# adaliaramon/LambdaGap

Measured on AMD Instinct MI355X. Metric: boosting iters/sec + AUC, synthetic Higgs-shape 10M×28, 255 bins, 63 leaves, higher is better.
Workload: dtype fp32; 1 GPU; model=gbdt binary, 63 leaves, 255 bins, lr 0.1, global_batch=10000000, seq_len=28, parallelism=dp1, device=AMD GPU (gfx950:sramecc+:xnack-) [frontier engine]

## Files before the change

src/device/device_learner.hip:

```cpp
#include <hip/hip_runtime.h>

#include <algorithm>
#include <chrono>
#include <cmath>
#include <cstdio>
#include <cstdlib>
#include <cstring>
#include <fstream>
#include <map>
#include <memory>
#include <string>
#include <vector>

#include "device/grad_kernels.h"
#include "device/hip_common.h"
#include "device/leaf_kernels.h"
#include "device/metric_kernels.h"
#include "device/linear_kernels.h"
#include "device/runtime_internal.h"
#include "device/frontier.h"
#include "device/policy_scan.h"
#include "device/traverse_kernels.h"
#include "device/sample_kernels.h"
#include "device/engine_plan.h"
#include "device/seq_kernels.h"
#include "device/split_scan.h"
#include "device/tree_kernels.h"
#include "learner/forced_splits.h"
#include "learner/linear_solve.h"
#include "learner/parallel_tree_learner.h"
#include "learner/serial_tree_learner.h"
#include "lgap/common.h"
#include "lgap/device_api.h"
#include "lgap/network.h"
#include "lgap/objective.h"
#include "lgap/rank_math.h"
#include "lgap/metric.h"
#include "lgap/split_math.h"

namespace lgap {
namespace device {
namespace {

const char* KernelOverride(const char* key) {
  static const char* const kKeys[] = {"fhist_threads", "hist_lds_kb", "quant_lds32", "part_iters",
                                      "hist_il",       "nibble",      "quant_hist",  "scan_global",
                                      "scan_wave",     "oob_rows",    "select_merge"};
  constexpr int kNumKeys = static_cast<int>(sizeof(kKeys) / sizeof(kKeys[0]));
  thread_local std::string vals[kNumKeys];
  const char* e = std::getenv("LGAP_KERNEL");
  if (e == nullptr) return nullptr;
  const std::string s(e);
  const char* found = nullptr;
  for (size_t p = 0; p < s.size();) {
    size_t q = s.find(',', p);
    if (q == std::string::npos) q = s.size();
    const std::string item = s.substr(p, q - p);
    p = q + 1;
    if (item.empty()) continue;
    const size_t eq = item.find('=');
    const std::string k = item.substr(0, eq);
    int idx = -1;
    for (int i = 0; i < kNumKeys; ++i) idx = k == kKeys[i] ? i : idx;
    if (idx < 0) Log::Fatal("LGAP_KERNEL: unknown key '%s'", k.c_str());
    if (k == key) {
      vals[idx] = eq == std::string::npos ? "1" : item.substr(eq + 1);
      found = vals[idx].c_str();
    }
  }
  return found;
}


using namespace seq;

template <typename T>
class PinnedBuf {
 public:
  ~PinnedBuf() {
    if (p_) (void)hipHostFree(p_);
// ... 1597 lines not shown
      facc_recv_.Resize(static_cast<size_t>(K) * bbin_ * 2);
    }
    if (plan_.bynode_on_device) {
      bool filt = false;
      const std::vector<uint8_t> m = col_sampler_.ByNodeSampleModes(&fbyn_cnt_, &filt);
      fbyn_reset_ = filt ? 1 : 0;
      fbyn_mode_.Resize(m.size());
      fbyn_mode_.Upload(m.data(), m.size(), stream_);
    }
    if (fvoting_) {
      SplitParams sl = MakeArgs().sp;
      sl.min_data_in_leaf = config_->min_data_in_leaf / P_;
      sl.min_sum_hessian_in_leaf = config_->min_sum_hessian_in_leaf / P_;
      fsp_local_.Resize(1);
      fsp_local_.Upload(&sl, 1, stream_);
      flsum_loc_.Resize(C);
      fltot_.Resize(2 * K);
      fltot_.Zero(stream_);
      fvrec_.Resize(static_cast<size_t>(P_) * 2 * K * topk_);
      fvelect_.Resize(2 * K * static_cast<size_t>(topk_ + 1));
      fvrows_.Resize(2 * K * static_cast<size_t>(topk_) * 2 * max_bin_);
    }
    fpart_iters_ = part_iters_;
    fpart_tile_ = kPartThreads * fpart_iters_;
    ftile_cap_ = DivUp(N_, fpart_tile_) + fkmax_ + 1;
    ftile_pub_.Resize(ftile_cap_);
    ftile_pub_.Zero(stream_);
    for (int i = 3; i < kFrontierIdx; ++i) idx_[i].Resize(std::max(N_, 1));
    {
      const int per_cu = std::max(1, FrontierPartitionBlocksPerCU(fpart_iters_));
      fpart_grid_ = std::max(1, std::min(ftile_cap_, per_cu * num_cu_));
    }
    fscan_lds_ = FrontierScanLds(max_bin_, has_cat_ ? max_cat_bin_ : 1);
    FrontierSetLds(FrontierHistLds(), fscan_lds_, use_dp_, width_);
    fspec_cap_ = 0;
    fhist_threads_ = big_tiles_ || (num_tiles_ == 1 && N_ >= 4000000) ? 1024 : 512;
    if (const char* e = KernelOverride("fhist_threads")) fhist_threads_ = std::atoi(e) == 1024 ? 1024 : 512;
    fpolicy_ = 1;
    fspec_alpha_ = 1.0;
    const char* spec_env = std::getenv("LGAP_FRONTIER_SPEC");
    const std::string spec = spec_env != nullptr ? spec_env : "";
    fspec_fixed_ = spec != "adapt";
    if (!spec.empty() && spec != "adapt" && spec != "fixed") {
      char* end = nullptr;
      const double alpha = std::strtod(spec.c_str(), &end);
      if (end == spec.c_str() || *end != '\0') Log::Fatal("LGAP_FRONTIER_SPEC=%s: expected fixed|adapt|<alpha>", spec.c_str());
      fspec_alpha_ = std::max(0.01, std::min(4.0, alpha));
    }
    {
      stune_ = SpecTuner();
      const char* te = std::getenv("LGAP_SPEC_TUNE");
      const bool tune_small = te == nullptr || te[0] != '0';
      stune_.on = !plan_.distributed && (L_ >= 128 || tune_small) && !plan_.raw_cands && fnum_forced_ == 0 &&
                  spec.empty();
      if (L_ < 128 && te == nullptr) stune_.rest = 64;
    }
    if (std::getenv("LGAP_FSTAMPS")) {
      fstamps_.Resize(256 * 4 * kFStampSlots);
      fstamps_.Zero(stream_);
    }
    for (auto& kv : fgraphs_) (void)hipGraphExecDestroy(kv.second);
    fgraphs_.clear();
    if (fcont_) (void)hipGraphExecDestroy(fcont_);
    fcont_ = nullptr;
  }

  FArgs MakeFArgs() const {
    FArgs a;
    std::memset(&a, 0, sizeof(a));
    a.rowbins = rowbins_.get();
// ... 58 lines not shown
    if (nib_) {
      a.rowbins = rowbins4_.get();
      a.stride_dw = stride4_dw_;
      a.tiles = ntile_.get();
      a.hist_nib = 1;
    }
    a.part_tile = fpart_tile_;
    a.max_depth = config_->max_depth;
    a.use_monotone = config_->monotone_constraints.empty() ? 0 : 1;
    a.mono_inter = fcbnd_ != nullptr ? 1 : 0;
    a.cbnd = fcbnd_;
    const char* sm = KernelOverride("select_merge");
    a.salive = sm != nullptr && sm[0] == '0' ? nullptr : fsal_;
    a.monotone_penalty = config_->monotone_penalty;
    a.cegb_split = CegbPenalty::Enabled(config_) ? config_->cegb_tradeoff * config_->cegb_penalty_split : 0.0;
    a.max_bin = max_bin_;
    a.cat_p2 = cat_p2_;
    a.use_dp = use_dp_ ? 1 : 0;
    a.ghq = ghq_.get();
    a.qmax = qmax_.get();
    a.quant = QuantHist() && ghq_.size() >= static_cast<size_t>(K_) * N_ ? 1 : 0;
    a.qbins = std::max(2, config_->num_grad_quant_bins);
    a.qconst = is_const_hess_ ? 1 : 0;
    {
      const double rows = static_cast<double>(N_);
      const double gl = a.qbins / 2, hl = a.qconst ? 1 : a.qbins;
      a.qpack = rows * gl < 2147483647.0 && rows * hl < 4294967295.0 ? 1 : 0;
      const int sub = static_cast<int>(std::min(32767.0 / gl, 65535.0 / hl));
      const char* e = KernelOverride("quant_lds32");
      const bool want = e != nullptr ? e[0] != '0' : num_tiles_ == 1;
      a.qsub = a.quant && !use_dp_ && sub >= 2048 && want ? sub : 0;
    }
    a.hist_il = !use_dp_ && a.qsub == 0 ? HistInterleave() : 0;
    {
      const bool fits = kFScanWaves * FrontierScanWaveBytes(max_bin_, cat_p2_) <= 150 * 1024;
      const char* sw = KernelOverride("scan_wave");
      a.scan_wave = fits && !has_cat_ && !a.mono_inter && (F_ >= 64 || (sw != nullptr && sw[0] == '1')) ? 1 : 0;
      a.scan_grid = 512;
    }
    a.e_lo = 0;
    a.e_hi = kFrontierKmax;
    if (plan_.raw_cands && fnuep_.size() > 0) {
      a.cegb_raw = 1;
      a.cegb_tradeoff = config_->cegb_tradeoff;
      a.nkey = fnkey_.get();
      a.ninfo = fninfo_.get();
      a.nuep = fnuep_.get();
      if (plan_.cegb_coupled) {
        a.cegb_coupled = cegb_coupled_.get();
        a.cegb_used = cegb_used_.get();
        a.cegb_epoch = cegb_epoch_.get();
      }
      if (plan_.cegb_lazy) {
        a.cegb_lazy = cegb_lazy_.get();
        a.lazy_bits = lazy_bits_.get();
        a.lazy_words = lazy_words_;
        a.lazy_acc = lazy_acc_.get();
        a.nlazy = fnlazy_.get();
        a.npath = fnpath_.get();
      }
    }
    a.spec_cap = fspec_cap_;
    a.policy = fpolicy_;
    a.stamps = fstamps_.size() ? fstamps_.get() : nullptr;
    a.distributed = plan_.distributed ? 1 : 0;
    a.kcap = fcaps_on_ ? fkcap_.get() : nullptr;
// ... 481 lines not shown
    if (renew && gh_true_.size() < static_cast<size_t>(N_)) gh_true_.Resize(N_);
    qmax_.Zero(stream_);
    const int grid = std::max(1, std::min(DivUp(N_, 256), num_cu_ * 4));
    k_qmax<<<grid, 256, 0, stream_>>>(gh, N_, qmax_.get());
    HIP_CHECK(hipGetLastError());
    if (Network::num_machines() > 1) {
      unsigned* hm = pin_max_.Get(2);
      qmax_.Download(hm, 2, stream_);
      HIP_CHECK(hipStreamSynchronize(stream_));
      float v[2];
      std::memcpy(v, hm, 8);
      v[0] = static_cast<float>(Network::GlobalSyncUpByMax(static_cast<double>(v[0])));
      v[1] = static_cast<float>(Network::GlobalSyncUpByMax(static_cast<double>(v[1])));
      std::memcpy(hm, v, 8);
      HIP_CHECK(hipMemcpyAsync(qmax_.get(), hm, 8, hipMemcpyHostToDevice, stream_));
    }
    const uint32_t seed = static_cast<uint32_t>(config_->seed) * 0x9E3779B9u + (quant_round_++);
    uint16_t* ghq = nullptr;
    if (QuantHist()) {
      if (ghq_.size() < static_cast<size_t>(K_) * N_) {
        ghq_.Resize(static_cast<size_t>(K_) * N_);
        InvalidateGraph();
      }
      ghq = ghq_.get() + static_cast<size_t>(class_id) * N_;
    }
    k_quantize<<<grid, 256, 0, stream_>>>(gh, renew ? gh_true_.get() : nullptr, ghq, N_, qmax_.get(),
                                          std::max(2, config_->num_grad_quant_bins), is_const_hess_ ? 1 : 0, seed,
                                          config_->stochastic_rounding ? 1 : 0);
    HIP_CHECK(hipGetLastError());
  }

  size_t FrontierHistLds() const {
    const FArgs fa = MakeFArgs();
    const size_t plan = use_dp_ || fa.qsub > 0 ? hist_lds_plain_ : hist_lds_bytes_;
    const size_t b = use_dp_ || !QuantHist() || fa.qsub == 0 ? plan : plan * 3 / 2 + 64;
    return b;
  }

  bool QuantHist() const {
    return config_->use_quantized_grad && std::max(2, config_->num_grad_quant_bins) <= 254 &&
           KernelOverride("quant_hist") == nullptr;
  }

  void RenewQuantizedLeaves(Tree* tree) {
    const int nl = tree->num_leaves();
    const Args args = MakeArgs();
    k_leaf_true_sums<<<nl, kNodeThreads, 0, stream_>>>(args, gh_true_.get(), nl, true_sums_.get());
    HIP_CHECK(hipGetLastError());
    std::vector<double2> st(nl);
    true_sums_.Download(st.data(), nl, stream_);
    HIP_CHECK(hipStreamSynchronize(stream_));
    std::vector<double> flat(2 * nl);
    for (int l = 0; l < nl; ++l) flat[2 * l] = st[l].x, flat[2 * l + 1] = st[l].y;
    if (plan_.distributed) Network::GlobalSum(&flat);
    SplitParams p = MakeArgs().sp;
    p.path_smooth = 0.0;
    for (int l = 0; l < nl; ++l) {
      tree->SetLeafOutput(l, LeafOutputRaw(flat[2 * l], flat[2 * l + 1], p, tree->leaf_count(l), 0.0));
    }
  }

  void BackendSetGradients(const float* g, const float* h, int n) {
    if (n != N_) Log::Fatal("HistogramBackend: %d gradients for %d rows", n, N_);
    K_ = 1;
    if (gh_.size() < static_cast<size_t>(N_)) gh_.Resize(static_cast<size_t>(N_));
    DeviceSetGradients(g, h, 1);
    float mg = 0.f, mh = 0.f;
    for (int i = 0; i < N_; ++i) {
      mg = std::max(mg, std::fabs(g[i]));
      mh = std::max(mh, std::fabs(h[i]));
// ... 559 lines not shown
    if (scan_global_) {
      scan_scratch_.Resize(scan_scratch_stride_ * static_cast<size_t>(std::max(F_, 1)));
      Log::Debug("HIP split scan: %d-bin features use %zu bytes of global scratch per block", max_bin_,
                 scan_scratch_stride_);
    } else if (scan_lds_bytes_ > 64 * 1024) {
      HIP_CHECK(hipFuncSetAttribute(reinterpret_cast<const void*>(k_reduce_scan<float, false>),
                                    hipFuncAttributeMaxDynamicSharedMemorySize, static_cast<int>(scan_lds_bytes_)));
      HIP_CHECK(hipFuncSetAttribute(reinterpret_cast<const void*>(k_reduce_scan<double, false>),
                                    hipFuncAttributeMaxDynamicSharedMemorySize, static_cast<int>(scan_lds_bytes_)));
    }
    std::vector<int> gs(std::max(G_, 1));
    for (int g = 0; g < G_; ++g) gs[g] = data_->group(g).hist_start;
    h_gstart_ = gs;
    BuildTiles();
    BuildNibbleRows();
    HIP_CHECK(hipStreamSynchronize(stream_));
  }

  void BuildTiles() {
    row_align_ = RowAlign();
    const int env_kb = [] {
      const char* e = KernelOverride("hist_lds_kb");
      return e ? std::max(16, std::min(150, std::atoi(e))) : 0;
    }();
    big_tiles_ = false;
    PlanTiles(env_kb > 0 ? env_kb * 1024 : kHistLdsBytes);
    if (env_kb == 0 && plan_.mode == ParallelMode::kSerial && num_tiles_ > 1 && min_tile_dw_ < 16) {
      big_tiles_ = true;
      PlanTiles(150 * 1024);
    }
    if (num_tiles_ > 1 && row_align_ > 0) PadTrainingRows(row_align_);
    if (num_tiles_ == 1) {
      if (N_ >= (4 << 20) && stride_dw_ > 4 && stride_dw_ < 8) PadTrainingRows(8);
    }
  }

  void BuildNibbleRows() {
    nib_ = false;
    const char* e = KernelOverride("nibble");
    if (e != nullptr && e[0] == '0') return;
    if (width_ != 1 || num_tiles_ != 1 || G_ <= 0 || N_ <= 0 || h_tiles_.empty() || h_tiles_[0].direct) return;
    for (int g = 0; g < G_; ++g) {
      if (data_->group(g).num_bin > 16) return;
    }
    stride4_dw_ = DivUp(G_, 8);
    rowbins4_.Resize(static_cast<size_t>(N_) * stride4_dw_);
    LaunchPackNibbles(rowbins_.get(), tstride_dw_, N_, G_, rowbins4_.get(), stride4_dw_, stream_);
    HistTile t = h_tiles_[0];
    t.d0 = 0;
    t.d1 = stride4_dw_;
    ntile_.Resize(1);
    ntile_.Upload(&t, 1, stream_);
    HIP_CHECK(hipStreamSynchronize(stream_));
    nib_ = true;
    Log::Debug("HIP learner: 4-bit rows (%d dwords per row instead of %d)", stride4_dw_, stride_dw_);
  }

  void PlanTiles(int lds_budget) {
    const int per = 4 / width_;
    const size_t acc = use_dp_ ? 16 : 8;
    const int max_bins = static_cast<int>(lds_budget / acc) - 64;
    const int max_dw = kHistThreads / 2;
    std::vector<HistTile> tiles;
    hist_lds_bytes_ = 16;
    hist_lds_plain_ = 16;
    int d = 0;
// ... 987 lines not shown
```

src/device/frontier.h:

```cpp
#pragma once

#include <hip/hip_runtime.h>

#include <cstdint>

#include "device/frontier_shape.h"
#include "device/tree_kernels.h"
#include "lgap/split_math.h"

namespace lgap {
namespace device {

#ifndef LGAP_FRONTIER_BUFS
#define LGAP_FRONTIER_BUFS 4
#endif
constexpr int kFrontierBufs = LGAP_FRONTIER_BUFS;
constexpr int kFrontierIdx = kFrontierBufs + 1;
constexpr int kFrontierRoundCap = 64;

__host__ __device__ inline int FixedPointExp(double limit, double rows, float vmax, float vsum) {
  double b = rows * static_cast<double>(vmax);
  if (static_cast<double>(vsum) < b) b = static_cast<double>(vsum);
  if (!(b > 0.0)) return 0;
  int e;
  (void)frexp(limit / b, &e);
  return e - 1;
}

__host__ __device__ inline int FrontierDepthBuf(int j) { return j < 2 ? j : j + 1; }

constexpr uint8_t kNodeExpanded = 1;
constexpr uint8_t kNodeCommitted = 2;
constexpr uint8_t kNodeDead = 4;
constexpr uint8_t kNodeStale = 0x40;
constexpr uint8_t kNodeEligTmp = 0x20;
constexpr uint8_t kNodeRescanTmp = 0x10;
constexpr uint8_t kNodeLocal = 0xF0;
constexpr int kFStampPart = 0, kFStampHist = 1, kFStampScan = 2, kFStampSel = 3, kFStampSlots = 8;

struct FNode {
  int buf, start, count;
  int gcount;
  int depth, parent;
  int left;
  int fidx;
};

struct FPairBest {
  SplitKey key;
  SplitInfo info;
};

struct FForced {
  int feature, threshold, left, right;
};

struct FExp {
  int parent, left, depth;
  int tile0, ntiles;
  int src_buf, start, count;
  int dst_buf;
  int group, offset, num_bin, mfb, default_bin, missing, thr, default_left, is_cat;
  int skip;
  int smaller, larger;
  int h_buf, h_start, h_count;
  int forced;
  int feature;
  int last;
  int rescan;
};

// ... 47 lines not shown
  double* slots;
  unsigned long long* acc;
  unsigned long long* hslab;
  size_t hslab_stride;
  long long* hmeta;
  int red_grid;
  int own, own_P, own_rank, own_w;
  const int* own_b0;
  unsigned long long* acc_recv;
  int xkb;
  const int* fown_list;
  int fown_n;
  const unsigned* ghmax;
  int sum_mult;
  int sum_bound;
  const FForced* forced;
  int num_forced;
  SplitInfo* fbest;
  SplitKey* fkey;
  const uint16_t* ghq;
  const unsigned* qmax;
  int quant;
  int qpack;
  int qbins, qconst;
  int qsub;
  SplitKey* ckey;
  SplitInfo* cinfo;
  unsigned long long* tile_pub;
  unsigned* bar;
  int part_selfcount;
  int hist_min_rows, hist_grid;
  int hist_threads;
  int hist_il;
  int scan_wave;
  int scan_grid;
  int hist_nib;
  int part_tile;
  int max_depth, use_monotone;
  int mono_inter;
  LeafBounds* cbnd;
  int* salive;
  double monotone_penalty;
  double cegb_split;
  const double* cegb_coupled;
  double cegb_tradeoff;
  uint8_t* cegb_used;
  unsigned* cegb_epoch;
  SplitKey* nkey;
  SplitInfo* ninfo;
  int* nuep;
  int cegb_raw;
  const double* cegb_lazy;
  uint32_t* lazy_bits;
  int lazy_words;
  int* lazy_acc;
  int* nlazy;
  uint32_t* npath;
  int max_bin, cat_p2;
  int use_dp;
  int spec_cap;
  int policy;
  int distributed;
  const int* kcap;
  int* kused;
  unsigned long long* stamps;
  int e_lo, e_hi;
// ... 81 lines not shown
```

src/device/frontier_kernels.hip:

```cpp
#include <hip/hip_runtime.h>

#include <algorithm>
#include <cstdint>

#include "device/frontier.h"
#include "device/hip_common.h"
#include "device/split_scan.h"
#include "lgap/split_math.h"

namespace lgap {
namespace device {
namespace {

constexpr int kFPartThreads = 256;
constexpr int kFScanThreads = 256;
constexpr int kFSelThreads = 1024;
#ifndef LGAP_FHIST_R
#define LGAP_FHIST_R 16
#endif

__device__ __forceinline__ int FRowAt(const FArgs& a, int buf, int pos) { return buf < 0 ? pos : a.idx[buf][pos]; }

__device__ __forceinline__ uint32_t FColBin(const FArgs& a, int g, int row) {
  const size_t o = static_cast<size_t>(g) * a.N + row;
  return a.width == 1 ? a.colbins[o] : reinterpret_cast<const uint16_t*>(a.colbins)[o];
}

__device__ __forceinline__ void FStamp(const FArgs& a, int r, int kern, int i) {
  if (a.stamps != nullptr && blockIdx.x == 0 && blockIdx.y == 0 && threadIdx.x == 0) {
    a.stamps[((static_cast<size_t>(r & 255) * 4 + kern) * kFStampSlots) + i] = wall_clock64();
  }
}
__device__ __forceinline__ void FStampMax(const FArgs& a, int r, int kern, int i) {
  if (a.stamps != nullptr && threadIdx.x == 0) {
    atomicMax(&a.stamps[((static_cast<size_t>(r & 255) * 4 + kern) * kFStampSlots) + i], wall_clock64());
  }
}
__device__ __forceinline__ void FStampEnd(const FArgs& a, int r, int kern) {
  if (a.stamps != nullptr && threadIdx.x == 0) {
    atomicMax(&a.stamps[((static_cast<size_t>(r & 255) * 4 + kern) * kFStampSlots) + 7], wall_clock64());
  }
}

__device__ __forceinline__ int Pow2Exp(double x) {
  int e;
  (void)frexp(x, &e);
  return e - 1;
}

__device__ __forceinline__ void GlobalScaleExp(const FArgs& a, int* eg, int* eh) {
  const double n = static_cast<double>(a.tp->root_gcount > 0 ? a.tp->root_gcount : 1);
  constexpr double k62 = 4611686018427387904.0;
  const float m = a.sum_bound ? static_cast<float>(a.sum_mult > 1 ? a.sum_mult : 1) : INFINITY;
  *eg = FixedPointExp(k62, n, __uint_as_float(a.ghmax[0]), __uint_as_float(a.ghmax[2]) * m);
  *eh = FixedPointExp(k62, n, __uint_as_float(a.ghmax[1]), __uint_as_float(a.ghmax[3]) * m);
}

__device__ __forceinline__ void QuantScales(const FArgs& a, double* gs, double* hs) {
// ... 201 lines not shown
#pragma unroll
    for (int j = 0; j < kRootStatsF; ++j) sh[j][w] = v[j];
  }
  __syncthreads();
  if (threadIdx.x == 0) {
    for (int i = 1; i < static_cast<int>(blockDim.x / 64); ++i) {
#pragma unroll
      for (int j = 0; j < kRootStatsF; ++j) v[j] = FRootFold(j, v[j], sh[j][i]);
    }
    a.lsum[0] = make_double2(v[0], v[1]);
    ghmax[0] = __float_as_uint(static_cast<float>(v[2]));
    ghmax[1] = __float_as_uint(static_cast<float>(v[3]));
    ghmax[2] = __float_as_uint(__double2float_ru(v[4] * (1.0 + 0x1p-20)));
    ghmax[3] = __float_as_uint(__double2float_ru(v[5] * (1.0 + 0x1p-20)));
  }
}

constexpr int kFHistR2 = LGAP_FHIST_R / 2;
__device__ __forceinline__ void FHistFirstRows(const FArgs& a, const HistTile& tile, int buf, int start, int rb, int re,
                                               int* rn) {
  const int tpr = tile.d1 - tile.d0;
  const int rpi = blockDim.x / tpr;
  const int myr = threadIdx.x / tpr;
  const int* idx = buf < 0 ? nullptr : a.idx[buf] + start;
  const int base = buf < 0 ? start : 0;
#pragma unroll
  for (int j = 0; j < kFHistR2; ++j) {
    const int p = rb + myr + j * rpi;
    rn[j] = myr < rpi && p < re ? (idx ? idx[p] : base + p) : -1;
  }
}

template <int W, int MODE>
__device__ __forceinline__ void FHistRows(const FArgs& a, const HistTile& tile, int buf, int start, int rb, int re,
                                          const int* gst, unsigned long long* hist, float sg, float sh, double dsg,
                                          double dsh, uint32_t* hist32 = nullptr, int il_gp = 0,
                                          const int* first_rows = nullptr) {
  const int tpr = tile.d1 - tile.d0;
  const int rpi = blockDim.x / tpr;
  const int myr = threadIdx.x / tpr;
  const int myd = threadIdx.x - myr * tpr;
  if (myr >= rpi) return;
  constexpr int per = W == 0 ? 8 : 4 / W;
  constexpr int R = LGAP_FHIST_R;
  const int dw = tile.d0 + myd;
  const int gfirst = dw * per;
  int go[per], gsh[per];
  const int rot = (MODE == 0 || MODE == 2) && il_gp > 0 ? (myr & (per - 1)) : 0;
#pragma unroll
  for (int kk = 0; kk < per; ++kk) {
    int gv = -1, sv = 0;
#pragma unroll
    for (int k = 0; k < per; ++k) {
      if (k == ((kk + rot) & (per - 1))) {
        const int gl = gfirst + k - tile.g0;
        gv = gfirst + k < tile.g1 ? (il_gp > 0 ? gl : gst[gl]) : -1;
        sv = (W == 0 ? 4 : W == 1 ? 8 : 16) * k;
      }
    }
    go[kk] = gv;
    gsh[kk] = sv;
  }
  const float2* gh = a.gh + static_cast<size_t>(a.tp->cls) * a.N;
  const uint16_t* ghq = MODE >= 2 ? a.ghq + static_cast<size_t>(a.tp->cls) * a.N : nullptr;
  const int* idx = buf < 0 ? nullptr : a.idx[buf] + start;
  const int base = buf < 0 ? start : 0;
  constexpr int R2 = R / 2;
  static_assert(R2 == kFHistR2, "first-chunk prefetch width");
  const int step = rpi * R2;
  auto load_rows = [&](int p0, int* rows) {
#pragma unroll
    for (int j = 0; j < R2; ++j) {
      const int p = p0 + j * rpi;
      rows[j] = p < re ? (idx ? idx[p] : base + p) : -1;
    }
  };
  auto load_data = [&](const int* rows, uint32_t* word, float2* v, uint32_t* q) {
#pragma unroll
    for (int j = 0; j < R2; ++j) {
      word[j] = rows[j] >= 0 ? a.rowbins[static_cast<size_t>(rows[j]) * a.stride_dw + dw] : 0u;
      if (MODE >= 2) q[j] = rows[j] >= 0 ? ghq[rows[j]] : 0u;
      else v[j] = rows[j] >= 0 ? gh[rows[j]] : make_float2(0.f, 0.f);
    }
  };
  int rn[R2];
  uint32_t word[R2], q[R2];
  float2 v[R2];
  if (first_rows != nullptr) {
#pragma unroll
    for (int j = 0; j < R2; ++j) rn[j] = first_rows[j];
  } else {
    load_rows(rb + myr, rn);
  }
  load_data(rn, word, v, q);
  load_rows(rb + myr + step, rn);
  for (int p0 = rb + myr; p0 < re; p0 += step) {
    uint32_t wn[R2], qn[R2];
    float2 vn[R2];
    load_data(rn, wn, vn, qn);
    load_rows(p0 + 2 * step, rn);
#pragma unroll
    for (int j = 0; j < R2; ++j) {
      unsigned long long pg = 0ull, ph = 0ull;
      uint32_t p32 = 0u;
      if (MODE == 3) {
        p32 = (static_cast<uint32_t>(static_cast<int32_t>(static_cast<int8_t>(q[j] >> 8))) << 16) + (q[j] & 0xFFu);
      } else if (MODE == 2) {
        const long long ig = static_cast<int8_t>(q[j] >> 8);
        pg = (static_cast<unsigned long long>(ig) << 32) + (q[j] & 0xFFu);
      } else if (MODE == 0) {
        const long long ig = __float2int_rn(v[j].x * sg);
        const long long ih = __float2int_rn(v[j].y * sh);
        pg = (static_cast<unsigned long long>(ig) << 32) + static_cast<unsigned long long>(ih);
      } else {
        pg = static_cast<unsigned long long>(__double2ll_rn(static_cast<double>(v[j].x) * dsg));
        ph = static_cast<unsigned long long>(__double2ll_rn(static_cast<double>(v[j].y) * dsh));
      }
#pragma unroll
      for (int k = 0; k < per; ++k) {
        const uint32_t b = (word[j] >> gsh[k]) & (W == 0 ? 0xFu : W == 1 ? 0xFFu : 0xFFFFu);
        if (b != 0u && go[k] >= 0) {
          const int o = il_gp > 0 ? static_cast<int>(b) * il_gp + go[k] : go[k] + static_cast<int>(b);
          if (MODE == 3) {
            atomicAdd(&hist32[o], p32);
          } else if (MODE != 1) {
            atomicAdd(&hist[o], pg);
          } else {
            atomicAdd(&hist[2 * o], pg);
            atomicAdd(&hist[2 * o + 1], ph);
          }
        }
      }
    }
#pragma unroll
    for (int j = 0; j < R2; ++j) {
      word[j] = wn[j];
      q[j] = qn[j];
      v[j] = vn[j];
    }
  }
}

struct FChunkSrc {
  int cnt, buf, start;
};
__device__ __forceinline__ FChunkSrc FHistChunkLoad(const FArgs& a) {
  FChunkSrc c{0, -1, 0};
  const int t = threadIdx.x;
  if (t < kFrontierKmax) {
    const FExp& x = a.exps[t];
    c.cnt = x.skip ? 0 : x.h_count;
    c.buf = x.h_buf;
    c.start = x.h_start;
  }
  return c;
}
__device__ __forceinline__ void FHistChunks(const FArgs& a, int k, const FChunkSrc& src, int* cnt, int* nb, int* inc) {
  const int t = threadIdx.x;
  *cnt = t < k && t >= a.e_lo && t < a.e_hi ? src.cnt : 0;
  const int total = WaveSum(*cnt);
  const int ke = WaveSum(*cnt > 0 ? 1 : 0);
  const int slots = max(max(1, a.hist_grid / 2), a.hist_grid - ke);
  const int c = max(a.hist_min_rows, (total + slots - 1) / slots);
  *nb = (*cnt + c - 1) / c;
  *inc = WaveInclusiveScan(*nb);
}

template <int W, int MODE, int THREADS>
__global__ __launch_bounds__(THREADS) void k_f_hist(FArgs a) {
  extern __shared__ __align__(8) unsigned char lds_raw[];
  __shared__ int s_e, s_rb, s_re, s_buf, s_start;
  const FState* sp = a.st;
  const int t = threadIdx.x;
  const FChunkSrc csrc = FHistChunkLoad(a);
  const HistTile tile = a.tiles[blockIdx.y];
  const int ng0 = tile.g1 - tile.g0;
  const int gst0 = t < ng0 ? a.gstart[tile.g0 + t] : 0;
  int EG, EH;
  GlobalScaleExp(a, &EG, &EH);
  if (sp->done) return;
  const int k = sp->k;
  const int rnd = sp->round;
  FStamp(a, rnd, kFStampHist, 0);
  if (t < 64) {
    int cnt, nb, inc;
    FHistChunks(a, k, csrc, &cnt, &nb, &inc);
    const int bx = static_cast<int>(blockIdx.x);
    const bool mine = nb > 0 && bx >= inc - nb && bx < inc;
    const unsigned long long m = __ballot(mine);
    if (mine) {
      const int j = bx - (inc - nb);
      const int chunk = (cnt + nb - 1) / nb;
      s_e = t;
      s_rb = j * chunk;
      s_re = min(cnt, (j + 1) * chunk);
      s_buf = csrc.buf;
      s_start = csrc.start;
    }
    if (t == 0 && m == 0ull) s_e = -1;
  }
  __syncthreads();
  const int e = s_e;
  if (e < 0) return;
// ... 55 lines not shown
                           : W == 1 ? ((word >> (8 * kk)) & 0xFFu)
                                    : ((word >> (16 * kk)) & 0xFFFFu);
        const int g = dw * per + kk;
        if (b != 0u && g < tile.g1) {
          unsigned long long* o = FAccPtr(a, e, gst[g - tile.g0] + static_cast<int>(b), pw);
          if (a.xg && a.own) {
            if (qg) FXAdd(o, qg);
            if (qh) FXAdd(o + 1, qh);
          } else {
            if (qg) atomicAdd(o, qg);
            if (qh) atomicAdd(o + 1, qh);
          }
        }
      }
    }
    if (a.xg && a.own) __builtin_amdgcn_s_waitcnt(0);
    return;
  }
  const double rows_in_block = static_cast<double>(re - rb > 0 ? re - rb : 1);
  constexpr double k30 = 1073741824.0;
  const float sbg = a.sum_bound ? __uint_as_float(a.ghmax[2]) : INFINITY;
  const float sbh = a.sum_bound ? __uint_as_float(a.ghmax[3]) : INFINITY;
  const int bg = FixedPointExp(k30, rows_in_block, __uint_as_float(a.ghmax[0]), sbg);
  const int bh = FixedPointExp(k30, rows_in_block, __uint_as_float(a.ghmax[1]), sbh);
  const float sg = ldexpf(1.f, bg), sh = ldexpf(1.f, bh);
  const int ng = tile.g1 - tile.g0;
  const int il_gp = (MODE == 0 || MODE == 2) && a.hist_il && tile.pad > 0 && (buf < 0 || a.hist_il > 1) ? ((ng + 15) & ~15) : 0;
  const int words = il_gp > 0 ? tile.pad * il_gp : (MODE != 1 ? tile.nbins : 2 * tile.nbins);
  unsigned long long* hist = reinterpret_cast<unsigned long long*>(lds_raw);
  uint32_t* hist32 = reinterpret_cast<uint32_t*>(hist + words);
  int* gst = reinterpret_cast<int*>(MODE == 3 ? reinterpret_cast<unsigned long long*>(hist32 + ((tile.nbins + 1) & ~1))
                                              : hist + words);
  unsigned long long* packed = il_gp > 0 ? reinterpret_cast<unsigned long long*>(gst + ((ng + 1) & ~1)) : nullptr;
  int first_rows[kFHistR2];
  if (MODE != 3) FHistFirstRows(a, tile, buf, start, rb, re, first_rows);
  for (int i = t; i < words; i += blockDim.x) hist[i] = 0ull;
  if (MODE == 3) {
    for (int i = t; i < tile.nbins; i += blockDim.x) hist32[i] = 0u;
  }
  for (int g = t; g < ng0; g += blockDim.x) gst[g] = (g == t ? gst0 : a.gstart[tile.g0 + g]) - tile.bin0;
  __syncthreads();
  FStamp(a, rnd, kFStampHist, 1);
  if (MODE == 3) {
    for (int sb = rb; sb < re; sb += a.qsub) {
      const int se = min(re, sb + a.qsub);
      FHistRows<W, MODE>(a, tile, buf, start, sb, se, gst, hist, sg, sh, dsg, dsh, hist32);
      __syncthreads();
      for (int i = t; i < tile.nbins; i += blockDim.x) {
        const uint32_t x = hist32[i];
        if (x == 0u) continue;
        hist32[i] = 0u;
        const uint32_t hs = x & 0xFFFFu;
        const long long gs = static_cast<int32_t>(x - hs) >> 16;
        hist[i] += (static_cast<unsigned long long>(gs) << 32) + hs;
      }
      __syncthreads();
    }
  } else {
    FHistRows<W, MODE>(a, tile, buf, start, rb, re, gst, hist, sg, sh, dsg, dsh, nullptr, il_gp, first_rows);
    __syncthreads();
  }
  if (il_gp > 0) {
    for (int sl = t; sl < words; sl += blockDim.x) {
      const int b = sl / il_gp, gl = sl - b * il_gp;
      if (gl >= ng) continue;
      const int nb = (gl + 1 < ng ? gst[gl + 1] : tile.nbins) - gst[gl];
      if (b < nb) packed[gst[gl] + b] = hist[sl];
    }
    __syncthreads();
  }
  FStamp(a, rnd, kFStampHist, 2);
  FStampMax(a, rnd, kFStampHist, 5);
  const int sw = MODE == 1 ? 2 : 1;
  unsigned long long* prow = a.hslab + static_cast<size_t>(blockIdx.x) * a.hslab_stride + static_cast<size_t>(sw) * tile.bin0;
  const unsigned long long* src = il_gp > 0 ? packed : hist;
  for (int j = t; j < sw * tile.nbins; j += blockDim.x) prow[j] = src[j];
  if (MODE == 0 && t == 0) {
    a.hmeta[blockIdx.x] = static_cast<long long>((static_cast<unsigned long long>(static_cast<unsigned>(bh)) << 32) |
                                                 static_cast<unsigned>(bg));
  }
  FStamp(a, rnd, kFStampHist, 3);
  FStampMax(a, rnd, kFStampHist, 6);
  FStampEnd(a, rnd, kFStampHist);
}

constexpr int kRedThreads = 256;
constexpr int kRedRows = 16;
constexpr int kRedMaxTiles = 256;

template <int MODE, bool XG>
__global__ __launch_bounds__(kRedThreads) void k_f_reduce(FArgs a) {
  __shared__ int s_nb[kFrontierKmax], s_b0[kFrontierKmax], s_w0[kFrontierKmax + 1];
// ... 433 lines not shown
        kk.feature = out->feature;
        kk.gain = SafeGain(*out);
        kk.threshold = out->threshold;
        kk.group = fi.group;
        kk.offset = fi.offset;
        kk.num_bin = fi.num_bin;
        kk.mfb = fi.mfb;
        kk.default_bin = fi.default_bin;
        kk.missing = fi.missing;
        kk.default_left = out->default_left;
        kk.is_cat = fi.bin_type != 0 ? 1 : 0;
        kk.pad0 = a.cegb_raw && out->feature >= 0 ? out->monotone_type : 0;
      }
    }
    __syncthreads();
    if (item == static_cast<int>(blockIdx.x)) FStamp(a, rnd, kFStampScan, 2);
    constexpr int kKeyWords = static_cast<int>(sizeof(SplitKey) / 4);
    constexpr int kInfoWords = static_cast<int>(sizeof(SplitInfo) / 4);
    const int nsel = cl >= 0 ? 2 : 1;
    for (int i = t; i < nsel * (kKeyWords + kInfoWords); i += blockDim.x) {
      const int sel = i / (kKeyWords + kInfoWords);
      const int o = i - sel * (kKeyWords + kInfoWords);
      const size_t q = (static_cast<size_t>(e) * 2 + sel) * F + f;
      if (o < kKeyWords) {
        reinterpret_cast<uint32_t*>(a.ckey + q)[o] = reinterpret_cast<const uint32_t*>(&s_key[sel])[o];
      } else {
        reinterpret_cast<uint32_t*>(a.cinfo + q)[o - kKeyWords] = reinterpret_cast<const uint32_t*>(&s_out[sel])[o - kKeyWords];
      }
    }
    __syncthreads();
    if (item == static_cast<int>(blockIdx.x)) FStamp(a, rnd, kFStampScan, 3);
  }
  FStampEnd(a, rnd, kFStampScan);
}

__device__ __forceinline__ void FWaveSync() {
  __builtin_amdgcn_fence(__ATOMIC_RELEASE, "workgroup");
  __builtin_amdgcn_wave_barrier();
  __builtin_amdgcn_fence(__ATOMIC_ACQUIRE, "workgroup");
}

__global__ __launch_bounds__(kFScanWaves * 64) void k_f_scan_w(FArgs a) {
  extern __shared__ __align__(16) unsigned char smem[];
  __shared__ __align__(8) unsigned char s_out_raw[kFScanWaves * sizeof(SplitInfo)];
  __shared__ SplitKey s_key[kFScanWaves];
  const FState* stp = a.st;
  if (stp->done) return;
  const int e0 = a.e_lo, e1 = min(stp->k, a.e_hi), F = a.F;
  const int total = max(0, e1 - e0) * F;
  const int rnd = stp->round;
  FStamp(a, rnd, kFStampScan, 0);
  const int t = threadIdx.x, lane = t & 63, w = t >> 6;
  int EG, EH;
  GlobalScaleExp(a, &EG, &EH);
  double inv_g = ldexp(1.0, -EG), inv_h = ldexp(1.0, -EH);
  if (a.quant) QuantScales(a, &inv_g, &inv_h);
  const bool qpack = a.quant && a.qpack;
  const size_t TB2 = 2 * static_cast<size_t>(a.TB);
  double* hs_full = reinterpret_cast<double*>(smem + w * FrontierScanWaveBytes(a.max_bin, a.cat_p2));
  double* hl_full = hs_full + 2 * a.max_bin;
  SplitInfo* out = reinterpret_cast<SplitInfo*>(s_out_raw) + w;
  SplitKey* key = &s_key[w];
  constexpr int kKeyWords = static_cast<int>(sizeof(SplitKey) / 4);
  constexpr int kInfoWords = static_cast<int>(sizeof(SplitInfo) / 4);
  for (int item = static_cast<int>(blockIdx.x) * kFScanWaves + w; item < total;
       item += static_cast<int>(gridDim.x) * kFScanWaves) {
    const int e = e0 + item / F, f = item - (e - e0) * F;
    const FExp& xr = a.exps[e];
    if (xr.skip) continue;
    const int cs = xr.smaller, cl = xr.larger, p = xr.parent;
    const DevFeature fi = a.feat[f];
    const int nbin = fi.num_bin;
// ... 2699 lines not shown
```

Baseline: 390.3 iters/s.

## Stage histogram row loads through per-wave LDS ring with 16-byte vector loads

Adds a staged histogram path for 8-bit bins in which each wave's lanes cooperatively load whole row segments as 16-byte vectors, plus gradient/hessian pairs, into a per-wave LDS ring. The lanes then read their own bin word from LDS and do the atomic adds, with wave-level fences between the two phases. Loads are software-pipelined with depth D. The aim is to replace narrow, poorly coalesced per-thread global loads of row bins with wide coalesced ones, at the cost of extra LDS space, wave syncs and possibly lower occupancy. It is on by default for single-tile datasets with at least 4M rows, which matches this workload.

After: 393.8 iters/s, median of 6. Within noise of the previous version (+0.9%).

```diff
diff --git a/src/device/device_learner.hip b/src/device/device_learner.hip
--- a/src/device/device_learner.hip
+++ b/src/device/device_learner.hip
@@ -45,7 +45,7 @@
 const char* KernelOverride(const char* key) {
   static const char* const kKeys[] = {"fhist_threads", "hist_lds_kb", "quant_lds32", "part_iters",
                                       "hist_il",       "nibble",      "quant_hist",  "scan_global",
-                                      "scan_wave",     "oob_rows",    "select_merge"};
+                                      "scan_wave",     "oob_rows",    "select_merge", "hist_stage"};
   constexpr int kNumKeys = static_cast<int>(sizeof(kKeys) / sizeof(kKeys[0]));
   thread_local std::string vals[kNumKeys];
   const char* e = std::getenv("LGAP_KERNEL");
@@ -1709,10 +1709,10 @@
       fpart_grid_ = std::max(1, std::min(ftile_cap_, per_cu * num_cu_));
     }
     fscan_lds_ = FrontierScanLds(max_bin_, has_cat_ ? max_cat_bin_ : 1);
-    FrontierSetLds(FrontierHistLds(), fscan_lds_, use_dp_, width_);
     fspec_cap_ = 0;
     fhist_threads_ = big_tiles_ || (num_tiles_ == 1 && N_ >= 4000000) ? 1024 : 512;
     if (const char* e = KernelOverride("fhist_threads")) fhist_threads_ = std::atoi(e) == 1024 ? 1024 : 512;
+    FrontierSetLds(FrontierHistLds(), fscan_lds_, use_dp_, width_);
     fpolicy_ = 1;
     fspec_alpha_ = 1.0;
     const char* spec_env = std::getenv("LGAP_FRONTIER_SPEC");
@@ -1837,6 +1837,7 @@
       a.qsub = a.quant && !use_dp_ && sub >= 2048 && want ? sub : 0;
     }
     a.hist_il = !use_dp_ && a.qsub == 0 ? HistInterleave() : 0;
+    a.hist_stage = HistStage(a.qsub) ? 1 : 0;
     {
       const bool fits = kFScanWaves * FrontierScanWaveBytes(max_bin_, cat_p2_) <= 150 * 1024;
       const char* sw = KernelOverride("scan_wave");
@@ -2384,10 +2385,26 @@
 
   size_t FrontierHistLds() const {
     const FArgs fa = MakeFArgs();
-    const size_t plan = use_dp_ || fa.qsub > 0 ? hist_lds_plain_ : hist_lds_bytes_;
-    const size_t b = use_dp_ || !QuantHist() || fa.qsub == 0 ? plan : plan * 3 / 2 + 64;
+    return FrontierHistLdsPlan(fa.qsub) + (fa.hist_stage ? FrontierHistStageLds(fhist_threads_) : 0);
+  }
+  size_t FrontierHistLdsPlan(int qsub) const {
+    const size_t plan = use_dp_ || qsub > 0 ? hist_lds_plain_ : hist_lds_bytes_;
+    const size_t b = use_dp_ || !QuantHist() || qsub == 0 ? plan : plan * 3 / 2 + 64;
     return b;
   }
+
+  bool HistStage(int qsub) const {
+    const char* e = KernelOverride("hist_stage");
+    if (e != nullptr && e[0] == '0') return false;
+    if (nib_ || width_ != 1 || tstride_dw_ % 4 != 0) return false;
+    constexpr size_t kCuLds = 160 * 1024, kBlockLds = 159 * 1024;
+    const size_t plan = FrontierHistLdsPlan(qsub), with = plan + FrontierHistStageLds(fhist_threads_);
+    if (with > kBlockLds) return false;
+    if (num_tiles_ > 1 && std::min<size_t>(kCuLds / with, 2) < std::min<size_t>(kCuLds / plan, 2)) return false;
+    if (e != nullptr) return true;
+    return HistStageDefault();
+  }
+  bool HistStageDefault() const { return num_tiles_ == 1 && N_ >= (4 << 20) && !use_dp_; }
 
   bool QuantHist() const {
     return config_->use_quantized_grad && std::max(2, config_->num_grad_quant_bins) <= 254 &&
@@ -3013,6 +3030,9 @@
     if (num_tiles_ > 1 && row_align_ > 0) PadTrainingRows(row_align_);
     if (num_tiles_ == 1) {
       if (N_ >= (4 << 20) && stride_dw_ > 4 && stride_dw_ < 8) PadTrainingRows(8);
+    }
+    if (const char* e = KernelOverride("hist_stage")) {
+      if (e[0] != '0' && width_ == 1 && tstride_dw_ % 4 != 0) PadTrainingRows(4);
     }
   }
 
diff --git a/src/device/frontier.h b/src/device/frontier.h
--- a/src/device/frontier.h
+++ b/src/device/frontier.h
@@ -37,6 +37,12 @@
 constexpr uint8_t kNodeRescanTmp = 0x10;
 constexpr uint8_t kNodeLocal = 0xF0;
 constexpr int kFStampPart = 0, kFStampHist = 1, kFStampScan = 2, kFStampSel = 3, kFStampSlots = 8;
+#ifndef LGAP_FHIST_STAGE_D
+#define LGAP_FHIST_STAGE_D 2
+#endif
+constexpr int kFHistStageD = LGAP_FHIST_STAGE_D;
+constexpr int kFHistStageWaveBytes = 1024 + 512;
+constexpr size_t FrontierHistStageLds(int threads) { return 32 + static_cast<size_t>(threads / 64) * kFHistStageWaveBytes; }
 
 struct FNode {
   int buf, start, count;
@@ -150,6 +156,7 @@
   int hist_min_rows, hist_grid;
   int hist_threads;
   int hist_il;
+  int hist_stage;
   int scan_wave;
   int scan_grid;
   int hist_nib;
diff --git a/src/device/frontier_kernels.hip b/src/device/frontier_kernels.hip
--- a/src/device/frontier_kernels.hip
+++ b/src/device/frontier_kernels.hip
@@ -24,6 +24,12 @@
 __device__ __forceinline__ uint32_t FColBin(const FArgs& a, int g, int row) {
   const size_t o = static_cast<size_t>(g) * a.N + row;
   return a.width == 1 ? a.colbins[o] : reinterpret_cast<const uint16_t*>(a.colbins)[o];
+}
+
+__device__ __forceinline__ void FWaveSync() {
+  __builtin_amdgcn_fence(__ATOMIC_RELEASE, "workgroup");
+  __builtin_amdgcn_wave_barrier();
+  __builtin_amdgcn_fence(__ATOMIC_ACQUIRE, "workgroup");
 }
 
 __device__ __forceinline__ void FStamp(const FArgs& a, int r, int kern, int i) {
@@ -291,6 +297,65 @@
 }
 
 template <int W, int MODE>
+__device__ __forceinline__ void FHistGroups(const HistTile& tile, const int* gst, int il_gp, int myr, int dw, int* go,
+                                            int* gsh) {
+  constexpr int per = W == 0 ? 8 : 4 / W;
+  const int gfirst = dw * per;
+  const int rot = (MODE == 0 || MODE == 2) && il_gp > 0 ? (myr & (per - 1)) : 0;
+#pragma unroll
+  for (int kk = 0; kk < per; ++kk) {
+    int gv = -1, sv = 0;
+#pragma unroll
+    for (int k = 0; k < per; ++k) {
+      if (k == ((kk + rot) & (per - 1))) {
+        const int gl = gfirst + k - tile.g0;
+        gv = gfirst + k < tile.g1 ? (il_gp > 0 ? gl : gst[gl]) : -1;
+        sv = (W == 0 ? 4 : W == 1 ? 8 : 16) * k;
+      }
+    }
+    go[kk] = gv;
+    gsh[kk] = sv;
+  }
+}
+
+template <int W, int MODE>
+__device__ __forceinline__ void FHistAdd(uint32_t word, float2 v, uint32_t q, const int* go, const int* gsh,
+                                         unsigned long long* hist, uint32_t* hist32, int il_gp, float sg, float sh,
+                                         double dsg, double dsh) {
+  constexpr int per = W == 0 ? 8 : 4 / W;
+  unsigned long long pg = 0ull, ph = 0ull;
+  uint32_t p32 = 0u;
+  if (MODE == 3) {
+    p32 = (static_cast<uint32_t>(static_cast<int32_t>(static_cast<int8_t>(q >> 8))) << 16) + (q & 0xFFu);
+  } else if (MODE == 2) {
+    const long long ig = static_cast<int8_t>(q >> 8);
+    pg = (static_cast<unsigned long long>(ig) << 32) + (q & 0xFFu);
+  } else if (MODE == 0) {
+    const long long ig = __float2int_rn(v.x * sg);
+    const long long ih = __float2int_rn(v.y * sh);
+    pg = (static_cast<unsigned long long>(ig) << 32) + static_cast<unsigned long long>(ih);
+  } else {
+    pg = static_cast<unsigned long long>(__double2ll_rn(static_cast<double>(v.x) * dsg));
+    ph = static_cast<unsigned long long>(__double2ll_rn(static_cast<double>(v.y) * dsh));
+  }
+#pragma unroll
+  for (int k = 0; k < per; ++k) {
+    const uint32_t b = (word >> gsh[k]) & (W == 0 ? 0xFu : W == 1 ? 0xFFu : 0xFFFFu);
+    if (b != 0u && go[k] >= 0) {
+      const int o = il_gp > 0 ? static_cast<int>(b) * il_gp + go[k] : go[k] + static_cast<int>(b);
+      if (MODE == 3) {
+        atomicAdd(&hist32[o], p32);
+      } else if (MODE != 1) {
+        atomicAdd(&hist[o], pg);
+      } else {
+        atomicAdd(&hist[2 * o], pg);
+        atomicAdd(&hist[2 * o + 1], ph);
+      }
+    }
+  }
+}
+
+template <int W, int MODE>
 __device__ __forceinline__ void FHistRows(const FArgs& a, const HistTile& tile, int buf, int start, int rb, int re,
                                           const int* gst, unsigned long long* hist, float sg, float sh, double dsg,
                                           double dsh, uint32_t* hist32 = nullptr, int il_gp = 0,
@@ -303,23 +368,8 @@
   constexpr int per = W == 0 ? 8 : 4 / W;
   constexpr int R = LGAP_FHIST_R;
   const int dw = tile.d0 + myd;
-  const int gfirst = dw * per;
   int go[per], gsh[per];
-  const int rot = (MODE == 0 || MODE == 2) && il_gp > 0 ? (myr & (per - 1)) : 0;
-#pragma unroll
-  for (int kk = 0; kk < per; ++kk) {
-    int gv = -1, sv = 0;
-#pragma unroll
-    for (int k = 0; k < per; ++k) {
-      if (k == ((kk + rot) & (per - 1))) {
-        const int gl = gfirst + k - tile.g0;
-        gv = gfirst + k < tile.g1 ? (il_gp > 0 ? gl : gst[gl]) : -1;
-        sv = (W == 0 ? 4 : W == 1 ? 8 : 16) * k;
-      }
-    }
-    go[kk] = gv;
-    gsh[kk] = sv;
-  }
+  FHistGroups<W, MODE>(tile, gst, il_gp, myr, dw, go, gsh);
   const float2* gh = a.gh + static_cast<size_t>(a.tp->cls) * a.N;
   const uint16_t* ghq = MODE >= 2 ? a.ghq + static_cast<size_t>(a.tp->cls) * a.N : nullptr;
   const int* idx = buf < 0 ? nullptr : a.idx[buf] + start;
@@ -360,42 +410,136 @@
     load_rows(p0 + 2 * step, rn);
 #pragma unroll
     for (int j = 0; j < R2; ++j) {
-      unsigned long long pg = 0ull, ph = 0ull;
-      uint32_t p32 = 0u;
-      if (MODE == 3) {
-        p32 = (static_cast<uint32_t>(static_cast<int32_t>(static_cast<int8_t>(q[j] >> 8))) << 16) + (q[j] & 0xFFu);
-      } else if (MODE == 2) {
-        const long long ig = static_cast<int8_t>(q[j] >> 8);
-        pg = (static_cast<unsigned long long>(ig) << 32) + (q[j] & 0xFFu);
-      } else if (MODE == 0) {
-        const long long ig = __float2int_rn(v[j].x * sg);
-        const long long ih = __float2int_rn(v[j].y * sh);
-        pg = (static_cast<unsigned long long>(ig) << 32) + static_cast<unsigned long long>(ih);
-      } else {
-        pg = static_cast<unsigned long long>(__double2ll_rn(static_cast<double>(v[j].x) * dsg));
-        ph = static_cast<unsigned long long>(__double2ll_rn(static_cast<double>(v[j].y) * dsh));
-      }
-#pragma unroll
-      for (int k = 0; k < per; ++k) {
-        const uint32_t b = (word[j] >> gsh[k]) & (W == 0 ? 0xFu : W == 1 ? 0xFFu : 0xFFFFu);
-        if (b != 0u && go[k] >= 0) {
-          const int o = il_gp > 0 ? static_cast<int>(b) * il_gp + go[k] : go[k] + static_cast<int>(b);
-          if (MODE == 3) {
-            atomicAdd(&hist32[o], p32);
-          } else if (MODE != 1) {
-            atomicAdd(&hist[o], pg);
-          } else {
-            atomicAdd(&hist[2 * o], pg);
-            atomicAdd(&hist[2 * o + 1], ph);
-          }
-        }
-      }
+      FHistAdd<W, MODE>(word[j], v[j], q[j], go, gsh, hist, hist32, il_gp, sg, sh, dsg, dsh);
     }
 #pragma unroll
     for (int j = 0; j < R2; ++j) {
       word[j] = wn[j];
       q[j] = qn[j];
       v[j] = vn[j];
+    }
+  }
+}
+
+typedef uint32_t FStagePiece __attribute__((ext_vector_type(4)));
+struct FStageGeo {
+  int q0;
+  int lpr;
+  int rps;
+  int G;
+};
+__device__ __forceinline__ FStageGeo FHistStageGeo(const HistTile& tile) {
+  FStageGeo s;
+  const int tpr = tile.d1 - tile.d0;
+  s.q0 = tile.d0 & ~3;
+  s.lpr = ((tile.d1 + 3) >> 2) - (tile.d0 >> 2);
+  s.rps = 64 / tpr;
+  s.G = (64 / s.lpr) / s.rps * s.rps;
+  return s;
+}
+__device__ __forceinline__ bool FHistStageTile(const FArgs& a, const HistTile& tile) {
+  return a.hist_stage != 0 && tile.d1 - tile.d0 <= 64;
+}
+__device__ __forceinline__ int FHistStagePos(const FStageGeo& s, int rb, int gi) {
+  const int wv = __builtin_amdgcn_readfirstlane(static_cast<int>(threadIdx.x >> 6));
+  return rb + (wv + gi * static_cast<int>(blockDim.x >> 6)) * s.G;
+}
+template <bool CONTIG>
+__device__ __forceinline__ int FHistStageRow(const FStageGeo& s, const int* idx, int base, int rb, int re, int gi) {
+  const int lr = static_cast<int>(threadIdx.x & 63) / s.lpr;
+  const int p = max(min(FHistStagePos(s, rb, gi) + min(lr, s.G - 1), re - 1), 0);
+  return CONTIG ? base + p : idx[p];
+}
+__device__ __forceinline__ void FHistStageFirstRows(const FArgs& a, const HistTile& tile, int buf, int start, int rb,
+                                                    int re, int* rn) {
+  const FStageGeo s = FHistStageGeo(tile);
+#pragma unroll
+  for (int j = 0; j < kFHistStageD; ++j) {
+    rn[j] = buf < 0 ? FHistStageRow<true>(s, nullptr, start, rb, re, j)
+                    : FHistStageRow<false>(s, a.idx[buf] + start, 0, rb, re, j);
+  }
+}
+
+template <int W, int MODE, bool CONTIG>
+__device__ __forceinline__ void FHistRowsStaged(const FArgs& a, const HistTile& tile, int buf, int start, int rb, int re,
+                                                const int* gst, unsigned long long* hist, float sg, float sh,
+                                                double dsg, double dsh, uint32_t* ring, uint32_t* hist32 = nullptr,
+                                                int il_gp = 0, const int* first_rows = nullptr) {
+  rb = __builtin_amdgcn_readfirstlane(rb);
+  re = __builtin_amdgcn_readfirstlane(re);
+  if (rb >= re) return;
+  constexpr int per = W == 0 ? 8 : 4 / W;
+  constexpr int D = kFHistStageD;
+  const FStageGeo s = FHistStageGeo(tile);
+  const int tpr = tile.d1 - tile.d0;
+  const int lane = threadIdx.x & 63;
+  const int wv = threadIdx.x >> 6, nw = blockDim.x >> 6;
+  const int lr = lane / s.lpr, lp = lane - lr * s.lpr;
+  const bool loader = lr < s.G;
+  const int myr = lane / tpr, myd = lane - myr * tpr;
+  const bool adder = myr < s.rps;
+  const int dw = tile.d0 + myd;
+  int go[per], gsh[per];
+  FHistGroups<W, MODE>(tile, gst, il_gp, myr, adder ? dw : tile.d0, go, gsh);
+  uint32_t* slot = ring + wv * (kFHistStageWaveBytes / 4);
+  FStagePiece* slot_rows = reinterpret_cast<FStagePiece*>(slot);
+  unsigned long long* slot_gh = reinterpret_cast<unsigned long long*>(slot + 256);
+  const int nsteps = s.G / s.rps;
+  const int row_dw = 4 * s.lpr;
+  const uint32_t* my_word = slot + myr * row_dw + (dw - s.q0);
+  const int step_dw = s.rps * row_dw;
+
+  const float2* gh = a.gh + static_cast<size_t>(a.tp->cls) * a.N;
+  const uint16_t* ghq = MODE >= 2 ? a.ghq + static_cast<size_t>(a.tp->cls) * a.N : nullptr;
+  const int* idx = CONTIG ? nullptr : a.idx[buf] + start;
+  const int base = CONTIG ? start : 0;
+  const uint32_t* my_piece = a.rowbins + s.q0 + 4 * lp;
+  auto load_row = [&](int row) {
+    return *reinterpret_cast<const FStagePiece*>(my_piece + static_cast<size_t>(row) * a.stride_dw);
+  };
+  auto load_gh = [&](int row) -> unsigned long long {
+    if (MODE >= 2) return ghq[row];
+    return *reinterpret_cast<const unsigned long long*>(gh + row);
+  };
+  int rn[D];
+  FStagePiece rw[D];
+  unsigned long long rv[D];
+#pragma unroll
+  for (int j = 0; j < D; ++j) {
+    rn[j] = first_rows != nullptr ? first_rows[j] : FHistStageRow<CONTIG>(s, idx, base, rb, re, j);
+  }
+#pragma unroll
+  for (int j = 0; j < D; ++j) {
+    rw[j] = load_row(rn[j]);
+    rv[j] = load_gh(rn[j]);
+    rn[j] = FHistStageRow<CONTIG>(s, idx, base, rb, re, D + j);
+    __builtin_amdgcn_sched_barrier(0);
+  }
+  for (int i = 0; FHistStagePos(s, rb, i) < re; i += D) {
+#pragma unroll
+    for (int j = 0; j < D; ++j) {
+      const int pos = FHistStagePos(s, rb, i + j);
+      const bool live = pos < re;
+      if (live && loader) {
+        slot_rows[lane] = rw[j];
+        if (lp == 0) slot_gh[lr] = rv[j];
+      }
+      rw[j] = load_row(rn[j]);
+      rv[j] = load_gh(rn[j]);
+      rn[j] = FHistStageRow<CONTIG>(s, idx, base, rb, re, i + j + 2 * D);
+      if (!live) continue;
+      FWaveSync();
+      if (adder) {
+        for (int st = 0; st < nsteps; ++st) {
+          const int r = st * s.rps + myr;
+          const uint32_t word = pos + r < re ? my_word[st * step_dw] : 0u;
+          const unsigned long long cell = slot_gh[r];
+          const uint32_t q = static_cast<uint32_t>(cell);
+          const float2 v = make_float2(__uint_as_float(q), __uint_as_float(static_cast<uint32_t>(cell >> 32)));
+          FHistAdd<W, MODE>(word, v, q, go, gsh, hist, hist32, il_gp, sg, sh, dsg, dsh);
+        }
+      }
+      FWaveSync();
     }
   }
 }
@@ -427,7 +571,7 @@
 
 template <int W, int MODE, int THREADS>
 __global__ __launch_bounds__(THREADS) void k_f_hist(FArgs a) {
-  extern __shared__ __align__(8) unsigned char lds_raw[];
+  extern __shared__ __align__(16) unsigned char lds_raw[];
   __shared__ int s_e, s_rb, s_re, s_buf, s_start;
   const FState* sp = a.st;
   const int t = threadIdx.x;
@@ -549,8 +693,17 @@
   int* gst = reinterpret_cast<int*>(MODE == 3 ? reinterpret_cast<unsigned long long*>(hist32 + ((tile.nbins + 1) & ~1))
                                               : hist + words);
   unsigned long long* packed = il_gp > 0 ? reinterpret_cast<unsigned long long*>(gst + ((ng + 1) & ~1)) : nullptr;
+  constexpr bool kStageable = W == 1;
+  const bool staged = kStageable && FHistStageTile(a, tile);
+  const int ring_off = (static_cast<int>(reinterpret_cast<unsigned char*>(gst + ((ng + 1) & ~1)) - lds_raw) + 15) & ~15;
+  uint32_t* ring = reinterpret_cast<uint32_t*>(lds_raw + ring_off);
   int first_rows[kFHistR2];
-  if (MODE != 3) FHistFirstRows(a, tile, buf, start, rb, re, first_rows);
+  int stage_rows[kFHistStageD];
+  if (staged) {
+    if (MODE != 3) FHistStageFirstRows(a, tile, buf, start, rb, re, stage_rows);
+  } else if (MODE != 3) {
+    FHistFirstRows(a, tile, buf, start, rb, re, first_rows);
+  }
   for (int i = t; i < words; i += blockDim.x) hist[i] = 0ull;
   if (MODE == 3) {
     for (int i = t; i < tile.nbins; i += blockDim.x) hist32[i] = 0u;
@@ -561,7 +714,11 @@
   if (MODE == 3) {
     for (int sb = rb; sb < re; sb += a.qsub) {
       const int se = min(re, sb + a.qsub);
-      FHistRows<W, MODE>(a, tile, buf, start, sb, se, gst, hist, sg, sh, dsg, dsh, hist32);
+      if (staged && buf < 0) {
+        FHistRowsStaged<W, MODE, true>(a, tile, buf, start, sb, se, gst, hist, sg, sh, dsg, dsh, ring, hist32);
+      } else if (staged) {
+        FHistRowsStaged<W, MODE, false>(a, tile, buf, start, sb, se, gst, hist, sg, sh, dsg, dsh, ring, hist32);
+      } else FHistRows<W, MODE>(a, tile, buf, start, sb, se, gst, hist, sg, sh, dsg, dsh, hist32);
       __syncthreads();
       for (int i = t; i < tile.nbins; i += blockDim.x) {
         const uint32_t x = hist32[i];
@@ -574,7 +731,15 @@
       __syncthreads();
     }
   } else {
-    FHistRows<W, MODE>(a, tile, buf, start, rb, re, gst, hist, sg, sh, dsg, dsh, nullptr, il_gp, first_rows);
+    if (staged && buf < 0) {
+      FHistRowsStaged<W, MODE, true>(a, tile, buf, start, rb, re, gst, hist, sg, sh, dsg, dsh, ring, nullptr, il_gp,
+                                     stage_rows);
+    } else if (staged) {
+      FHistRowsStaged<W, MODE, false>(a, tile, buf, start, rb, re, gst, hist, sg, sh, dsg, dsh, ring, nullptr, il_gp,
+                                      stage_rows);
+    } else {
+      FHistRows<W, MODE>(a, tile, buf, start, rb, re, gst, hist, sg, sh, dsg, dsh, nullptr, il_gp, first_rows);
+    }
     __syncthreads();
   }
   if (il_gp > 0) {
@@ -1074,12 +1239,6 @@
     if (item == static_cast<int>(blockIdx.x)) FStamp(a, rnd, kFStampScan, 3);
   }
   FStampEnd(a, rnd, kFStampScan);
-}
-
-__device__ __forceinline__ void FWaveSync() {
-  __builtin_amdgcn_fence(__ATOMIC_RELEASE, "workgroup");
-  __builtin_amdgcn_wave_barrier();
-  __builtin_amdgcn_fence(__ATOMIC_ACQUIRE, "workgroup");
 }
 
 __global__ __launch_bounds__(kFScanWaves * 64) void k_f_scan_w(FArgs a) {
```
